# ChanghyeonKim93/nonlinear_optimizer_for_slam

Measured on AMD Instinct MI355X. Metric: ndt6_gauss_newton_residual_blocks_per_sec, higher is better.
Workload: dtype f64

## Files before the change

### nonlinear_optimizer_for_slam_amd/csrc/assemble_one_launch.hpp

```cpp
#pragma once

#include "assemble_pass.hpp"

namespace nos {

constexpr size_t kSingleBlockMaxElements = size_t(1024) * 15;

template <typename Problem, typename T, int BLOCK, bool NT>
__device__ __forceinline__ int single_block_loop(const TiledLayout& L, typename Problem::Params& P, uint32_t n_chunks,
                                                 LmDevice& s_lm, double* s_sum, double* __restrict__ cost_history,
                                                 int history_capacity) {
  constexpr int kF = Problem::kFields;
  constexpr int kOut = Problem::kOut;
  const T* __restrict__ base = static_cast<const T*>(L.base);
  int executed = 0;
  while (s_lm.st.done == 0) {
    set_pose(P, &s_lm);
    T acc[kOut];
#pragma unroll
    for (int k = 0; k < kOut; ++k) acc[k] = T(0);
    constexpr uint32_t kRound = (kF * sizeof(T) > 64) ? 2 : 4;
    for (uint32_t c = 0; c < n_chunks; c += kRound) {
      T x[kRound][kF][1];
      uint64_t i0[kRound];
// ... 79 lines not shown
constexpr uint32_t kClusterMaxBlocks = 256;
constexpr unsigned long long kClusterTimeoutTicks = 5000000ull;
constexpr unsigned long long kClusterMailboxTimeoutTicks = kMailboxTimeoutTicks;

struct ClusterCtl {
  unsigned int abort;
  unsigned int pad0[31];
  struct alignas(128) Arrival {
    unsigned int count;
    unsigned int pad[31];
  } arrival[8];
};

__device__ __forceinline__ double sc1_load(const double* p) {
  return __hip_atomic_load(p, __ATOMIC_RELAXED, __HIP_MEMORY_SCOPE_AGENT);
}
__device__ __forceinline__ void sc1_store(double* p, double v) {
  __hip_atomic_store(p, v, __ATOMIC_RELAXED, __HIP_MEMORY_SCOPE_AGENT);
}

__device__ __forceinline__ void state_store_sc1(LmDevice* lm, const nos_host::LmState& st) {
  double* d = reinterpret_cast<double*>(&lm->st);
  const double* s = reinterpret_cast<const double*>(&st);
  constexpr int kWords = int(sizeof(nos_host::LmState) / sizeof(double));
  static_assert(sizeof(nos_host::LmState) % sizeof(double) == 0, "LmState must be a whole number of doubles");
#pragma unroll
  for (int k = 0; k < kWords; ++k) sc1_store(d + k, s[k]);
}
__device__ __forceinline__ void state_load_sc1(const LmDevice* lm, nos_host::LmState& st) {
  const double* d = reinterpret_cast<const double*>(&lm->st);
  double* s = reinterpret_cast<double*>(&st);
  constexpr int kWords = int(sizeof(nos_host::LmState) / sizeof(double));
#pragma unroll
  for (int k = 0; k < kWords; ++k) s[k] = sc1_load(d + k);
}

template <int FIELDS, int ELEM>
struct ResidentShape;
template <>
struct ResidentShape<15, 8> { static constexpr int RI = 3, LI = 3; };
template <>
struct ResidentShape<15, 4> { static constexpr int RI = 3, LI = 4; };
template <>
struct ResidentShape<5, 8> { static constexpr int RI = 9, LI = 7; };
template <>
struct ResidentShape<5, 4> { static constexpr int RI = 10, LI = 14; };

template <typename Problem, typename T>
struct StreamRegRounds { static constexpr int kRR = 3; };
template <int LOSS>
struct StreamRegRounds<Ndt6Problem<float, LOSS>, float> { static constexpr int kRR = 0; };
constexpr int kStreamRegRoundsMax = 3;

template <typename Problem, typename T, int BLOCK, int RI, int LI, int SI = 0, bool SPF = false, bool NT = false>
__global__ __launch_bounds__(BLOCK) void solve_cluster_kernel(TiledLayout L, typename Problem::Params P,
                                                             double* __restrict__ partials, LmDevice* lm, ClusterCtl* ctl,
                                                             double* __restrict__ cost_history, int history_capacity,
                                                             double* entry_host, unsigned long long* seq_host,
                                                             unsigned long long seq, uint32_t items_per_lane,
                                                             const Mailbox* mail = nullptr, uint32_t stream_lds = 0u,
                                                             uint32_t stream_reg = 0u) {
  constexpr int kF = Problem::kFields;
  constexpr int kOut = Problem::kOut;
  constexpr int kCols = 32;
  constexpr int kSlices = BLOCK / kCols;
  const T* __restrict__ base = static_cast<const T*>(L.base);
  constexpr int kRF = kF;
  extern __shared__ __align__(16) unsigned char resident_raw[];
  T* resident = reinterpret_cast<T*>(resident_raw);
  __shared__ int s_flag;
  __shared__ int s_fast;
  __shared__ double red[kSlices][kCols];
  __shared__ double s_tot[kLmTotDoubles(kOut)];
  __shared__ double s_lmd_raw[(sizeof(LmDevice) + 7) / 8];
  LmDevice& s_lmd = *reinterpret_cast<LmDevice*>(s_lmd_raw);
  nos_host::LmState& s_state = s_lmd.st;
  [[maybe_unused]] __shared__ double s_local[kCols];
  [[maybe_unused]] __shared__ unsigned long long s_round0;
  const bool multi = mail != nullptr;

  const uint32_t J = items_per_lane & 0x7fffffffu;
  [[maybe_unused]] const bool allow_fast = (items_per_lane >> 31) == 0u;
  [[maybe_unused]] constexpr int kXccCol = 28;
  [[maybe_unused]] const unsigned int my_xcc = xcc_id();
  const uint64_t block_base = uint64_t(blockIdx.x) * BLOCK * J;
  auto fetch = [&](uint32_t j, T (&dst)[kRF]) -> bool {
    const uint64_t i = block_base + uint64_t(j) * BLOCK + threadIdx.x;
    const bool ok = i < L.n;
    const uint64_t ic = ok ? i : 0;
    const uint64_t off = (ic >> L.tile_shift) * L.tile_stride + (ic & L.tile_mask);
    T xt[kF][1];
#pragma unroll
    for (int f = 0; f < kF; ++f) load_items<T, 1, false>(base + field_offset<Problem>(L, ic, off, f), xt[f]);
#pragma unroll
    for (int f = 0; f < kF; ++f) dst[f] = ok ? xt[f][0] : T(0);
    return ok;
  };
  auto evaluate_resident = [&](const T (&xi)[kRF], bool ok, T (&acc_)[kOut]) { Problem::item(xi, P, ok, acc_); };
  T x[RI > 0 ? RI : 1][kRF];
  bool valid[RI > 0 ? RI : 1];
  static_assert(SI == 0 || (RI == 0 && LI == 0), "the streaming form keeps nothing resident");
  constexpr int kSI = SI > 0 ? SI : 1;
  [[maybe_unused]] T xs[kF][kSI];
  [[maybe_unused]] uint64_t xs_i0 = 0;
  [[maybe_unused]] constexpr int kRR = (SI > 0 && !SPF) ? StreamRegRounds<Problem, T>::kRR : 0;
  static_assert(kRR <= kStreamRegRoundsMax, "the option's range covers every instantiation");
  [[maybe_unused]] T xr[kRR > 0 ? kRR : 1][kF][kSI];
  [[maybe_unused]] const uint32_t my_rounds = blockIdx.x < J ? (J - blockIdx.x + gridDim.x - 1) / gridDim.x : 0u;
  [[maybe_unused]] const uint32_t lds_k = SI > 0 ? min(stream_lds, my_rounds > 0u ? my_rounds - 1u : 0u) : 0u;
  [[maybe_unused]] const uint32_t reg_k = kRR > 0 ? min(min(stream_reg, uint32_t(kRR)), (my_rounds > 0u ? my_rounds - 1u : 0u) - lds_k) : 0u;
  [[maybe_unused]] const uint32_t alt_k = min(lds_k, reg_k);
  [[maybe_unused]] auto chip_round = [&](uint32_t i) -> uint32_t {
    return uint32_t(uint64_t(i + 1u) * my_rounds / (lds_k + reg_k + 1u));
  };
  [[maybe_unused]] auto lds_slot_round = [&](uint32_t sl) -> uint32_t {
    return sl < lds_k ? chip_round(sl < alt_k ? 2u * sl : alt_k + sl) : ~0u;
  };
  [[maybe_unused]] const uint32_t lds_r0 = lds_slot_round(0u);
  [[maybe_unused]] const uint32_t lds_r1 = lds_slot_round(1u);
  [[maybe_unused]] const uint32_t lds_r2 = lds_slot_round(2u);
  [[maybe_unused]] uint32_t reg_r[kRR > 0 ? kRR : 1];
#pragma unroll
  for (int j = 0; j < (kRR > 0 ? kRR : 1); ++j)
    reg_r[j] = uint32_t(j) < reg_k ? chip_round(uint32_t(j) < alt_k ? 2u * uint32_t(j) + 1u : alt_k + uint32_t(j)) : ~0u;
#pragma unroll
  for (int j = 0; j < (kRR > 0 ? kRR : 1); ++j)
#pragma unroll
    for (int f = 0; f < kF; ++f)
#pragma unroll
      for (int e = 0; e < kSI; ++e) xr[j][f][e] = T(0);
  [[maybe_unused]] auto lds_round = [&](uint32_t s) -> uint32_t { return s == 0u ? lds_r0 : s == 1u ? lds_r1 : s == 2u ? lds_r2 : ~0u; };
  [[maybe_unused]] auto fetch_chunk = [&](uint32_t c, T (&dst)[kF][kSI]) -> uint64_t {
    const uint64_t i0 = uint64_t(c) * (uint64_t(BLOCK) * kSI) + uint64_t(threadIdx.x) * kSI;
    const uint64_t off = (i0 >> L.tile_shift) * L.tile_stride + (i0 & L.tile_mask);
#pragma unroll
    for (int f = 0; f < kF; ++f) load_items<T, kSI, NT>(base + field_offset<Problem>(L, i0, off, f), dst[f]);
    return i0;
  };
  if constexpr (SI > 0) {
    if (blockIdx.x < J) xs_i0 = fetch_chunk(blockIdx.x, xs);
  }
#pragma unroll
  for (int j = 0; j < RI; ++j) {
    valid[j] = false;
    if (uint32_t(j) < J) {
      valid[j] = fetch(uint32_t(j), x[j]);
    } else {
#pragma unroll
      for (int f = 0; f < kRF; ++f) x[j][f] = T(0);
    }
  }
  if constexpr (LI > 0) {
    for (uint32_t j = RI; j < J; ++j) {
      T xi[kRF];
      (void)fetch(j, xi);
#pragma unroll
      for (int f = 0; f < kRF; ++f) resident[(size_t(j - RI) * kRF + f) * BLOCK + threadIdx.x] = xi[f];
    }
  }
  NOS_PROBE(if (threadIdx.x < 4) s_step_cycles[threadIdx.x] = 0ull;)
  if (threadIdx.x == 0) {
    s_lmd.settings = lm->settings;
    s_state = lm->st;
    s_flag = s_state.done != 0 ? 1 : 0;
    s_fast = 0;
    if (__hip_atomic_load(&ctl->abort, __ATOMIC_RELAXED, __HIP_MEMORY_SCOPE_AGENT) != 0u) s_flag = 2;
    if (multi && blockIdx.x == 0) s_round0 = *mail->round;
  }
  __syncthreads();
  [[maybe_unused]] const unsigned int group = blockIdx.x & 7u;
  const unsigned int n_groups = gridDim.x < 8u ? gridDim.x : 8u;
  unsigned int it = 0;
  int executed = 0;
  NOS_PROBE(unsigned long long tq[6] = {0, 0, 0, 0, 0, 0}, tp = 0;)
#define NOS_RES_STAMP(slot_) NOS_PROBE({ const unsigned long long now_ = wall_clock64(); tq[slot_] += now_ - tp; tp = now_; })
  while (s_flag == 0) {
    NOS_PROBE(tp = wall_clock64();)
    if constexpr (kOut == 28) {
#pragma unroll
      for (int k = 0; k < 9; ++k) P.R[k] = T(uniform_load(&s_state.R[k]));
#pragma unroll
      for (int k = 0; k < 3; ++k) P.t[k] = T(uniform_load(&s_state.t[k]));
    } else {
#pragma unroll
      for (int k = 0; k < 4; ++k) P.R2[k] = T(uniform_load(&s_state.R[k]));
#pragma unroll
      for (int k = 0; k < 2; ++k) P.t2[k] = T(uniform_load(&s_state.t[k]));
    }
    T acc[kOut];
#pragma unroll
    for (int k = 0; k < kOut; ++k) acc[k] = T(0);
    if constexpr (SI > 0) {
      const uint32_t n_chunks = J;
      auto evaluate = [&](const T (&xc)[kF][SI > 0 ? SI : 1], uint64_t i0) {
#pragma unroll
        for (int it = 0; it < (SI > 0 ? SI : 1); ++it) {
          T xi[kF];
#pragma unroll
          for (int f = 0; f < kF; ++f) xi[f] = xc[f][it];
          Problem::item(xi, P, (i0 + it) < L.n, acc);
        }
      };
      if constexpr (SPF) {
        for (uint32_t c = blockIdx.x; c < n_chunks; c += gridDim.x) {
          T xb[kF][SI > 0 ? SI : 1];
          uint64_t i1 = 0;
          const uint32_t cn = c + gridDim.x;
          if (cn < n_chunks) i1 = fetch_chunk(cn, xb);
          evaluate(xs, xs_i0);
#pragma unroll
          for (int f = 0; f < kF; ++f)
#pragma unroll
            for (int it = 0; it < (SI > 0 ? SI : 1); ++it) xs[f][it] = xb[f][it];
          xs_i0 = i1;
        }
      } else {
        auto lds_at = [&](uint32_t s, int f, int e) -> T& {
          return resident[((size_t(s) * kF + f) * BLOCK + threadIdx.x) * kSI + e];
        };
        auto evaluate_lds = [&](uint32_t s, uint32_t cl) {
          const uint64_t i0 = uint64_t(cl) * (uint64_t(BLOCK) * kSI) + uint64_t(threadIdx.x) * kSI;
#pragma unroll
          for (int e = 0; e < kSI; ++e) {
            T xi[kF];
#pragma unroll
            for (int f = 0; f < kF; ++f) xi[f] = lds_at(s, f, e);
            Problem::item(xi, P, (i0 + e) < L.n, acc);
          }
        };
        const bool on_chip = it != 0u;
        uint32_t s = 0;
        uint32_t next_res = lds_round(0u);
        auto in_registers = [&](uint32_t r) -> bool {
          bool hit = false;
#pragma unroll
          for (int j = 0; j < kRR; ++j) hit = hit || r == reg_r[j];
          return hit;
        };
        uint32_t k = 0;
        if constexpr (kRR == 0) {
          while (k < my_rounds) {
            __builtin_amdgcn_sched_barrier(0);
            if (!on_chip && k == next_res) {
#pragma unroll
              for (int f = 0; f < kF; ++f)
#pragma unroll
                for (int e = 0; e < kSI; ++e) lds_at(s, f, e) = xs[f][e];
              next_res = lds_round(++s);
            }
            evaluate(xs, xs_i0);
            uint32_t kn = k + 1u;
            if (on_chip)
              for (uint32_t sn = s; kn == lds_round(sn); ++sn) ++kn;
            xs_i0 = fetch_chunk(blockIdx.x + (kn < my_rounds ? kn : 0u) * gridDim.x, xs);
            for (uint32_t kr = k + 1u; kr < kn; ++kr) {
              evaluate_lds(s, blockIdx.x + kr * gridDim.x);
              next_res = lds_round(++s);
            }
            k = kn;
          }
        } else
#pragma unroll
        for (int j = 0; j <= kRR; ++j) {
          const uint32_t rj = j < kRR ? reg_r[j < kRR ? j : 0] : ~0u;
          const uint32_t stop = min(rj, my_rounds);
          const uint32_t hi = (!on_chip && rj != ~0u) ? rj + 1u : stop;
          auto lds_rounds_below = [&](uint32_t lim) {
            while (next_res < lim) {
              evaluate_lds(s, blockIdx.x + next_res * gridDim.x);
              next_res = lds_round(++s);
            }
          };
          if (on_chip && j > 0) lds_rounds_below(min(k, stop));
          while (k < hi) {
            __builtin_amdgcn_sched_barrier(0);
            if (!on_chip) {
              if (k == next_res) {
#pragma unroll
                for (int f = 0; f < kF; ++f)
#pragma unroll
                  for (int e = 0; e < kSI; ++e) lds_at(s, f, e) = xs[f][e];
                next_res = lds_round(++s);
              }
              if constexpr (kRR > 0) {
                if (j < kRR && k == rj) {
#pragma unroll
                  for (int f = 0; f < kF; ++f)
#pragma unroll
                    for (int e = 0; e < kSI; ++e) xr[j < kRR ? j : 0][f][e] = xs[f][e];
                }
              }
            }
            evaluate(xs, xs_i0);
            uint32_t kn = k + 1u;
            if (on_chip) {
              for (uint32_t sn = s;;) {
                if (kn == lds_round(sn)) {
                  ++sn;
                  ++kn;
                } else if (in_registers(kn)) {
                  ++kn;
                } else {
                  break;
                }
              }
            }
            xs_i0 = fetch_chunk(blockIdx.x + (kn < my_rounds ? kn : 0u) * gridDim.x, xs);
            if (on_chip) lds_rounds_below(min(kn, stop));
            k = kn;
          }
          if constexpr (kRR > 0) {
            if (j < kRR && on_chip && rj != ~0u)
              evaluate(xr[j < kRR ? j : 0], uint64_t(blockIdx.x + rj * gridDim.x) * (uint64_t(BLOCK) * kSI) + uint64_t(threadIdx.x) * kSI);
          }
        }
      }
      if constexpr (SPF) {
        if (blockIdx.x < n_chunks) xs_i0 = fetch_chunk(blockIdx.x, xs);
      }
    } else
    if (sizeof(T) == 8 && J >= uint32_t(RI)) {
#pragma unroll
      for (int j = 0; j < RI; ++j) evaluate_resident(x[j], valid[j], acc);
    } else {
#pragma unroll
      for (int j = 0; j < RI; ++j)
        if (uint32_t(j) < J) evaluate_resident(x[j], valid[j], acc);
    }
    if constexpr (LI > 0) {
      for (uint32_t j = RI; j < J; ++j) {
        T xi[kRF];
#pragma unroll
        for (int f = 0; f < kRF; ++f) xi[f] = resident[(size_t(j - RI) * kRF + f) * BLOCK + threadIdx.x];
        evaluate_resident(xi, (block_base + uint64_t(j) * BLOCK + threadIdx.x) < L.n, acc);
      }
    }
    double dacc[kOut];
#pragma unroll
    for (int k = 0; k < kOut; ++k) dacc[k] = double(acc[k]);
    NOS_RES_STAMP(0)
    {
      TaggedUnit* const block_units = reinterpret_cast<TaggedUnit*>(partials);
      TaggedUnit* const group_units = block_units + size_t(kClusterMaxBlocks) * 32;
      const unsigned long long tag = (seq << 24) | ((unsigned long long)it + 1ull);
      const double mine = block_reduce_value<kOut, BLOCK>(dacc);
      const bool probe = it == 0u && allow_fast;
      if (threadIdx.x < kOut) {
        if (s_fast != 0)
          tagged_store_plain(block_units + size_t(blockIdx.x) * 32 + threadIdx.x, mine, tag);
        else
          tagged_store(block_units + size_t(blockIdx.x) * 32 + threadIdx.x, mine, tag);
      } else if (probe && threadIdx.x == kXccCol) {
        tagged_store(block_units + size_t(blockIdx.x) * 32 + kXccCol, double(my_xcc), tag);
      }
      NOS_RES_STAMP(1)
      const unsigned long long deadline = wall_clock64() + (multi ? kClusterMailboxTimeoutTicks : kClusterTimeoutTicks);
      auto await = [&](const TaggedUnit* u, double* value) -> bool {
        unsigned int polls = 0;
        for (;;) {
          const TaggedUnit got = tagged_load(u);
          if (got.seq == tag) {
            *value = got.value;
            return true;
          }
          if ((++polls & 63u) == 0u &&
              (__hip_atomic_load(&ctl->abort, __ATOMIC_RELAXED, __HIP_MEMORY_SCOPE_AGENT) != 0u || wall_clock64() > deadline)) {
            __hip_atomic_store(&ctl->abort, 1u, __ATOMIC_RELAXED, __HIP_MEMORY_SCOPE_AGENT);
// ... 73 lines not shown
                const unsigned long long* slot_r = own + (size_t(r) * 2 + parity) * kMailSlotDoubles;
                unsigned long long got = 0ull;
                unsigned int polls = 0;
                for (;;) {
                  if (lane < 2 * kOut) got = __hip_atomic_load(slot_r + lane, __ATOMIC_RELAXED, __HIP_MEMORY_SCOPE_SYSTEM);
                  const bool here = lane >= 2 * kOut || (unsigned int)(got >> 32) == xtag;
                  if (__ballot(!here) == 0ull) break;
                  if ((++polls & 15u) == 0u) {
                    const unsigned long long peer_gave_up =
                        __hip_atomic_load(slot_r + 63, __ATOMIC_RELAXED, __HIP_MEMORY_SCOPE_SYSTEM);
                    if ((unsigned int)(peer_gave_up >> 32) == xtag || wall_clock64() > give_up_at ||
                        __hip_atomic_load(&ctl->abort, __ATOMIC_RELAXED, __HIP_MEMORY_SCOPE_AGENT) != 0u) {
                      lost = true;
                      break;
                    }
                  }
                  __builtin_amdgcn_s_sleep(1);
                }
                const unsigned int half = (unsigned int)(got & 0xFFFFFFFFull);
                const unsigned int other = (unsigned int)__shfl_xor(int(half), 1, kWave);
                const double value = __longlong_as_double((long long)(((unsigned long long)((lane & 1) ? half : other) << 32) |
                                                                      (unsigned long long)((lane & 1) ? other : half)));
                sum += value;
              }
              if (lost) {
                if (lane == 0) {
                  __hip_atomic_store(&ctl->abort, 1u, __ATOMIC_RELAXED, __HIP_MEMORY_SCOPE_AGENT);
                  s_flag = 2;
                }
                if (lane < mb.n_ranks)
                  __hip_atomic_store(reinterpret_cast<unsigned long long*>(mb.peers[lane] + units_base) +
                                         (size_t(mb.rank) * 2 + parity) * kMailSlotDoubles + 63,
                                     (unsigned long long)xtag << 32, __ATOMIC_RELAXED, __HIP_MEMORY_SCOPE_SYSTEM);
              } else if (lane < 2 * kOut && (lane & 1) == 0) {
                s_local[lane >> 1] = sum;
              }
            }
          }
          __syncthreads();
          if (s_flag != 2) {
            if (threadIdx.x < kOut || (probe && threadIdx.x == kXccCol))
              tagged_store(global_units + size_t(it & 1u) * 32 + threadIdx.x, s_local[threadIdx.x], tag);
          }
        }
        {
          double v = 0.0;
          if (threadIdx.x < kCols && (col < kOut || (probe && col == kXccCol)) && s_flag != 2)
            (void)await(global_units + size_t(it & 1u) * 32 + col, &v);
          if (threadIdx.x < kCols) red[0][col] = v;
        }
        __syncthreads();
      }
      NOS_RES_STAMP(2)
      if (s_flag == 2) break;
      if (multi) {
        if (threadIdx.x < kOut)
          s_tot[threadIdx.x] = red[0][threadIdx.x];
        else if (probe && threadIdx.x == kXccCol)
          s_fast = red[0][kXccCol] == 0.0 ? 1 : 0;
      } else
      if (threadIdx.x < kOut) {
        double tot = 0.0;
        for (unsigned int g = 0; g < n_groups; ++g) tot += red[g][threadIdx.x];
        s_tot[threadIdx.x] = tot;
      } else if (probe && threadIdx.x == kXccCol) {
        double strangers = 0.0;
        for (unsigned int g = 0; g < n_groups; ++g) strangers += red[g][kXccCol];
        s_fast = strangers == 0.0 ? 1 : 0;
      }
      __syncthreads();
    }
    {
      NOS_RES_STAMP(3)
      if (threadIdx.x == 0) {
        if (blockIdx.x == 0 && cost_history != nullptr && executed < history_capacity)
          __hip_atomic_store(cost_history + executed, s_tot[kOut - 1], __ATOMIC_RELAXED, __HIP_MEMORY_SCOPE_SYSTEM);
        lm_step_lane<kOut>(lds_ptr(s_tot), lds_ptr(&s_lmd));
        s_flag = s_state.done != 0 ? 1 : 0;
      }
    }
    ++executed;
    ++it;
    __syncthreads();
    NOS_RES_STAMP(4)
  }
  NOS_PROBE(
  if (blockIdx.x == 0 && threadIdx.x == 0 && entry_host != nullptr) {
    for (int k = 0; k < 5; ++k)
      __hip_atomic_store(entry_host + 50 + k, double(tq[k]) / double(executed > 0 ? executed : 1), __ATOMIC_RELAXED,
                         __HIP_MEMORY_SCOPE_SYSTEM);
    for (int k = 0; k < 3; ++k)
      __hip_atomic_store(entry_host + 56 + k, double(s_step_cycles[k]) / double(executed > 0 ? executed : 1), __ATOMIC_RELAXED,
                         __HIP_MEMORY_SCOPE_SYSTEM);
  }
  )
  if (s_flag == 1 && blockIdx.x == 0) {
    if (threadIdx.x < kOut && entry_host != nullptr && executed > 0)
      __hip_atomic_store(entry_host + kLogOut + threadIdx.x, s_tot[threadIdx.x], __ATOMIC_RELAXED, __HIP_MEMORY_SCOPE_SYSTEM);
    if (threadIdx.x == 0) {
      const nos_host::LmState st = s_state;
      lm->st = st;
      if (multi) *mail->round = s_round0 + (unsigned long long)executed;
      if (entry_host != nullptr) {
#pragma unroll
        for (int k = 0; k < 9; ++k)
          __hip_atomic_store(entry_host + kLogR + k, st.R[k], __ATOMIC_RELAXED, __HIP_MEMORY_SCOPE_SYSTEM);
#pragma unroll
        for (int k = 0; k < 3; ++k)
          __hip_atomic_store(entry_host + kLogT + k, st.t[k], __ATOMIC_RELAXED, __HIP_MEMORY_SCOPE_SYSTEM);
        __hip_atomic_store(entry_host + kLogLambda, st.lambda, __ATOMIC_RELAXED, __HIP_MEMORY_SCOPE_SYSTEM);
        __hip_atomic_store(entry_host + kLogPrevCost, st.previous_cost, __ATOMIC_RELAXED, __HIP_MEMORY_SCOPE_SYSTEM);
        __hip_atomic_store(entry_host + kLogCost, st.cost, __ATOMIC_RELAXED, __HIP_MEMORY_SCOPE_SYSTEM);
        __hip_atomic_store(entry_host + kLogIteration, double(st.iteration), __ATOMIC_RELAXED, __HIP_MEMORY_SCOPE_SYSTEM);
        __hip_atomic_store(entry_host + kLogDone, double(st.done), __ATOMIC_RELAXED, __HIP_MEMORY_SCOPE_SYSTEM);
        __hip_atomic_store(entry_host + kLogOk, double(st.ok), __ATOMIC_RELAXED, __HIP_MEMORY_SCOPE_SYSTEM);
        __hip_atomic_store(entry_host + kLogExecuted, double(executed), __ATOMIC_RELAXED, __HIP_MEMORY_SCOPE_SYSTEM);
      }
    }
    if (threadIdx.x < kWave) {
      asm volatile("s_waitcnt vmcnt(0)" ::: "memory");
      if (threadIdx.x == 0 && seq_host != nullptr) {
        __builtin_amdgcn_fence(__ATOMIC_RELEASE, "");
        asm volatile("s_waitcnt vmcnt(0)" ::: "memory");
        __hip_atomic_store(seq_host, seq, __ATOMIC_RELAXED, __HIP_MEMORY_SCOPE_SYSTEM);
      }
    }
  }
}

}
```

### nonlinear_optimizer_for_slam_amd/csrc/nos_core.hip

```cpp
#include "nos_internal.hpp"

namespace nosd {


thread_local const void* t_last_kernel = nullptr;

template <typename Problem, typename T, int ITEMS, int BLOCK, int MINW, int PREFETCH = 0>
int launch_variant(const nos::TiledLayout& L, const typename Problem::Params& P, int grid_cap, int num_cus_hint,
                   bool nt, double* partials, const nos::FusedFinal& fin_in, hipStream_t stream, int* rows_out) {
  constexpr uint32_t kChunk = BLOCK * ITEMS;
  if (L.n_padded % kChunk != 0) return fail(NOS_ERR_INVALID_ARGUMENT, "n_padded %% chunk != 0");
  if (L.tile_stride != 0 && ((size_t(L.tile_mask) + 1) % kChunk) != 0)
    return fail(NOS_ERR_INVALID_ARGUMENT, "tile not a multiple of the kernel chunk");
  const uint64_t n_chunks64 = L.n_padded / kChunk;
  if (n_chunks64 > 0xFFFFFFFFull) return fail(NOS_ERR_UNSUPPORTED, "dataset too large for one shard");
  const uint32_t n_chunks = uint32_t(n_chunks64);
  int grid = int(std::min<uint64_t>(n_chunks, uint64_t(grid_cap)));
  if (grid < 1) grid = 1;
  if (grid > kMaxPartialRows) grid = kMaxPartialRows;
  nos::FusedFinal fin = fin_in;
  fin.write_through = (fin.counter != nullptr && grid <= num_cus_hint && fin_in.write_through != 0) ? 1 : 0;
  const auto kernel = nt ? nos::assemble_kernel<Problem, T, ITEMS, BLOCK, MINW, true, PREFETCH>
                         : nos::assemble_kernel<Problem, T, ITEMS, BLOCK, MINW, false, PREFETCH>;
  t_last_kernel = reinterpret_cast<const void*>(kernel);
// ... 25 lines not shown
  if constexpr (sizeof(T) == 8) {
    if (variant == 0 && kReproj) variant = 7;
    switch (variant) {
      NOS_CASE(0, 1, 512, 3, 1)
      NOS_CASE(1, 1, 256, 3, 2)
      NOS_CASE(3, 2, 256, 2, 2)
      NOS_CASE_PP(7, 1, 512, kReproj ? 3 : 2, 1)
#ifdef NOS_ALL_VARIANTS
      NOS_CASE(2, 1, 256, 2, 2)
      NOS_CASE(4, 2, 512, 2, 1)
      NOS_CASE_PP(8, 2, 512, 2, 1)
#endif
    }
  } else {
    if (variant == 0) variant = kReproj ? 11 : 1;
    switch (variant) {
      NOS_CASE(1, 2, 512, 2, 1)
      NOS_CASE_PP(11, 2, 512, 2, 1)
#ifdef NOS_ALL_VARIANTS
      NOS_CASE(2, 1, 256, 4, 2)
      NOS_CASE(3, 2, 256, 5, 2)
      NOS_CASE(4, 2, 256, 4, 2)
      NOS_CASE(5, 1, 1024, 4, 1)
      NOS_CASE(6, 2, 1024, 4, 1)
      NOS_CASE(9, 2, 256, 3, 3)
      NOS_CASE_PP(12, 4, 512, 2, 1)
      NOS_CASE(13, 4, 256, 2, 1)
#endif
    }
  }
#undef NOS_CASE
#undef NOS_CASE_PP
  return fail(NOS_ERR_UNSUPPORTED, "launch geometry %d is not compiled into this build for this element type "
              "(default build: fp64 0, 1, 3, 7; fp32 1, 11; `make ALL_VARIANTS=1` builds the rest)", variant);
}

size_t resident_items_per_lane(int n_fields, int dtype) {
  if (n_fields == 15)
    return dtype == NOS_F64 ? size_t(nos::ResidentShape<15, 8>::RI + nos::ResidentShape<15, 8>::LI)
                            : size_t(nos::ResidentShape<15, 4>::RI + nos::ResidentShape<15, 4>::LI);
  if (n_fields == 5)
    return dtype == NOS_F64 ? size_t(nos::ResidentShape<5, 8>::RI + nos::ResidentShape<5, 8>::LI)
                            : size_t(nos::ResidentShape<5, 4>::RI + nos::ResidentShape<5, 4>::LI);
  return 1;
}

struct SingleBlockArgs {
  int cluster_blocks = 0;
  int items_per_lane = 1;
  int stream_chunks = 0;
  bool nt = false;
  int stream_lds_chunks = 0;
  int stream_reg_rounds = 0;
  bool stage1_sc1 = false;
  const nos::Mailbox* mail = nullptr;
  double* partials = nullptr;
  nos::ClusterCtl* ctl = nullptr;
  nos::LmDevice* lm;
  double* history;
  int history_capacity;
  double* entry;
  unsigned long long* seq_host;
  unsigned long long seq;
};

template <typename Problem, typename T>
int launch_single(const nos::TiledLayout& L, const typename Problem::Params& P, const SingleBlockArgs& a, hipStream_t stream) {
  constexpr int kBlock = 512;
  if (L.n_padded % kBlock != 0) return fail(NOS_ERR_INVALID_ARGUMENT, "n_padded %% 512 != 0");
  if (a.cluster_blocks > 0 && a.stream_chunks > 0) {
    constexpr int kSI = sizeof(T) == 8 ? 1 : 2;
    constexpr bool kSPF = false;
    constexpr size_t kChunk = size_t(kBlock) * kSI;
    if (L.n_padded % kChunk != 0 || (L.tile_stride != 0 && ((size_t(L.tile_mask) + 1) % kChunk) != 0))
      return fail(NOS_ERR_INVALID_ARGUMENT, "streaming solve: layout not a multiple of the %zu-item chunk", kChunk);
    if (size_t(a.stream_chunks) * kChunk != L.n_padded) return fail(NOS_ERR_INVALID_ARGUMENT, "streaming solve: chunk count does not match the layout");
    const auto kernel = a.nt ? nos::solve_cluster_kernel<Problem, T, kBlock, 0, 0, kSI, kSPF, true>
                             : nos::solve_cluster_kernel<Problem, T, kBlock, 0, 0, kSI, kSPF, false>;
    uint32_t lds = uint32_t(std::min(std::max(a.stream_lds_chunks, 0), 3));
    size_t dyn_bytes = lds * size_t(Problem::kFields) * kChunk * sizeof(T);
    if (dyn_bytes > size_t(48) * 1024 &&
        hipFuncSetAttribute(reinterpret_cast<const void*>(kernel), hipFuncAttributeMaxDynamicSharedMemorySize,
                            int(dyn_bytes)) != hipSuccess) {
      (void)hipGetLastError();
      lds = 0;
      dyn_bytes = 0;
    }
    const uint32_t reg = uint32_t(std::min(std::max(a.stream_reg_rounds, 0), nos::kStreamRegRoundsMax));
    t_last_kernel = reinterpret_cast<const void*>(kernel);
    hipLaunchKernelGGL(kernel, dim3(a.cluster_blocks), dim3(kBlock), dyn_bytes, stream, L, P, a.partials, a.lm, a.ctl, a.history,
                       a.history_capacity, a.entry, a.seq_host, a.seq, uint32_t(a.stream_chunks) | (a.stage1_sc1 ? 0x80000000u : 0u),
                       a.mail, lds, reg);
    hipError_t e = hipGetLastError();
    if (e != hipSuccess) return fail(NOS_ERR_HIP, "streaming solve launch failed: %s", hipGetErrorString(e));
    return NOS_OK;
  }
  if (a.cluster_blocks > 0) {
    using Shape = nos::ResidentShape<Problem::kPlanes, int(sizeof(T))>;
    if (a.items_per_lane < 1 || a.items_per_lane > Shape::RI + Shape::LI)
      return fail(NOS_ERR_INVALID_ARGUMENT, "resident solve: %d items per lane do not fit (%d + %d)", a.items_per_lane,
                  Shape::RI, Shape::LI);
    const auto kernel = nos::solve_cluster_kernel<Problem, T, kBlock, Shape::RI, Shape::LI>;
    const size_t lds_items = a.items_per_lane > Shape::RI ? size_t(a.items_per_lane - Shape::RI) : 0;
    const size_t dyn_bytes = lds_items * size_t(Problem::kFields) * kBlock * sizeof(T);
    if (dyn_bytes > size_t(48) * 1024) {
      const hipError_t ea = hipFuncSetAttribute(reinterpret_cast<const void*>(kernel),
                                                hipFuncAttributeMaxDynamicSharedMemorySize, int(dyn_bytes));
      if (ea != hipSuccess) return fail(NOS_ERR_UNSUPPORTED, "resident solve: %zu bytes of LDS refused: %s", dyn_bytes, hipGetErrorString(ea));
    }
    t_last_kernel = reinterpret_cast<const void*>(kernel);
    hipLaunchKernelGGL(kernel, dim3(a.cluster_blocks), dim3(kBlock), dyn_bytes, stream, L, P, a.partials, a.lm, a.ctl,
                       a.history, a.history_capacity, a.entry, a.seq_host, a.seq,
                       uint32_t(a.items_per_lane) | (a.stage1_sc1 ? 0x80000000u : 0u), a.mail, 0u, 0u);
    hipError_t e = hipGetLastError();
    if (e != hipSuccess) return fail(NOS_ERR_HIP, "cluster solve launch failed: %s", hipGetErrorString(e));
    return NOS_OK;
  }
  const uint32_t n_chunks = uint32_t((std::max<uint64_t>(L.n, 1) + kBlock - 1) / kBlock);
  t_last_kernel = reinterpret_cast<const void*>(&nos::solve_single_block_kernel<Problem, T, kBlock>);
  hipLaunchKernelGGL((nos::solve_single_block_kernel<Problem, T, kBlock>), dim3(1), dim3(kBlock), 0, stream, L, P, n_chunks, a.lm,
                     a.history, a.history_capacity, a.entry, a.seq_host, a.seq);
  hipError_t e = hipGetLastError();
  if (e != hipSuccess) return fail(NOS_ERR_HIP, "single-workgroup solve launch failed: %s", hipGetErrorString(e));
  return NOS_OK;
}

template <template <typename, int> class ProblemT, typename T, typename ParamsT>
int launch_by_loss(int loss_kind, int variant, int blocks_per_cu, int num_cus,
                   const nos::TiledLayout& L, const ParamsT& P, bool nt, double* partials,
                   const nos::FusedFinal& fin, hipStream_t stream, int* rows_out, const SingleBlockArgs* single = nullptr) {
  return with_loss(loss_kind, [&](auto loss) {
    using Problem = ProblemT<T, decltype(loss)::value>;
    if (single) return launch_single<Problem, T>(L, P, *single, stream);
    return launch_by_variant<Problem, T>(variant, blocks_per_cu, num_cus, L, P, nt, partials, fin, stream, rows_out);
  });
}

int check_loss(const nos_loss* loss, int* kind_out) {
  int kind = loss ? loss->kind : NOS_LOSS_NONE;
  if (kind < NOS_LOSS_NONE || kind > NOS_LOSS_HUBER) return fail(NOS_ERR_INVALID_ARGUMENT, "unknown loss kind %d", kind);
  if (kind == NOS_LOSS_EXPONENTIAL && (loss->a < 0.0 || loss->b < 0.0))
    return fail(NOS_ERR_INVALID_ARGUMENT, "exponential loss needs c1 >= 0 and c2 >= 0");
  if (kind == NOS_LOSS_HUBER && !(loss->a > 0.0)) return fail(NOS_ERR_INVALID_ARGUMENT, "huber loss needs threshold > 0");
  *kind_out = kind;
  return NOS_OK;
}

bool use_nontemporal(const nos_dataset* ds, const Shard& sh) {
  const int force = ds->ctx->settings.nt;
  if (force >= 0) return force != 0;
  return sh.bytes > (size_t(192) << 20);
}

template <template <typename, int> class ProblemT, typename T>
int launch_flat(const nos_dataset* ds, const Shard& sh, const Request& rq, double* partials, const nos::FusedFinal& fin,
                hipStream_t stream, int* rows_out, const SingleBlockArgs* single) {
  const nos_ctx* ctx = ds->ctx;
  typename ProblemT<T, nos::kLossNone>::Params P{};
  fill_params(P, rq, ds);
  return launch_by_loss<ProblemT, T>(rq.loss_kind, ctx->variant, ctx->blocks_per_cu, ctx->slots[sh.slot].num_cus, sh.layout, P,
                                     use_nontemporal(ds, sh), partials, fin, stream, rows_out, single);
}

int launch_assemble_inner(const nos_dataset* ds, const Shard& sh, const Request& rq, double* partials,
                          const nos::FusedFinal& fin_in, hipStream_t stream, int* rows_out, const SingleBlockArgs* single) {
  nos::FusedFinal fin = fin_in;
// ... 316 lines not shown
  const int executed = int(e[nos::kLogExecuted]);
  if (slot.prof_on && slot.prof_every == 0) slot.prof_launches += executed;
  copy_history(opt, slot, executed);
  return NOS_OK;
}

bool cluster_eligible(const nos_dataset* ds, const nos_lm_options* opt, bool mailbox_in_launch, size_t cluster_blocks,
                      bool resident_fits, bool stream_form, bool paused) {
  const nos_ctx* ctx = ds->ctx;
  const bool with_comm = ctx->comm != nullptr;
  return ds->kind != kKindNdtIndexed && !with_comm && (ctx->shm_dev == nullptr || mailbox_in_launch) && opt->max_iterations > 0 &&
         cluster_blocks >= 1 && (resident_fits || stream_form) && !paused &&
         ctx->settings.lm_cluster != 0 && (opt->cost_history == nullptr || opt->max_iterations <= kHistCapacity);
}

int solve_cluster(nos_dataset* ds, const Request& rq, const nos_lm_options* opt, const nos::LmInitArgs& init,
                  nos_host::LmState* st, bool* finished, int* fell_back) {
  nos_ctx* ctx = ds->ctx;
  const Shard& sh = ds->shards[0];
  DeviceSlot& slot = ctx->slots[sh.slot];
  *finished = false;
  const size_t max_blocks = std::min<size_t>(std::min<size_t>(nos::kClusterMaxBlocks, size_t(slot.num_cus)),
                                             size_t(std::max(1, ctx->settings.lm_cluster_max_blocks)));
  const bool mailbox_in_launch = ctx->shm_dev != nullptr && ctx->d_peers != nullptr && ctx->d_mail != nullptr &&
                                 ds->kind != kKindNdtIndexed;
  const size_t cluster_blocks = std::min<size_t>(max_blocks, (sh.layout.n + 511) / 512);
  const size_t items_per_lane = cluster_blocks > 0 ? (sh.layout.n + cluster_blocks * 512 - 1) / (cluster_blocks * 512) : 0;
  const size_t resident_capacity = ctx->settings.lm_cluster == 2 ? 1 : resident_items_per_lane(ds->n_fields, ds->dtype);
  const size_t stream_chunk = size_t(512) * (ds->dtype == NOS_F64 ? 1 : 2);
  const bool resident_fits = items_per_lane >= 1 && items_per_lane <= resident_capacity;
  const bool stream_form = !resident_fits && (ctx->settings.lm_cluster == 1 || ctx->settings.lm_cluster == 5) && items_per_lane >= 1 &&
                           sh.layout.n_padded % stream_chunk == 0 && sh.layout.n_padded / stream_chunk < (size_t(1) << 31) &&
                           (sh.layout.tile_stride == 0 || (size_t(sh.layout.tile_mask) + 1) % stream_chunk == 0);
  bool paused = false;
  if (mailbox_in_launch) {
    paused = slot.cluster_paused_solves > 0;
    if (paused) --slot.cluster_paused_solves;
  } else {
    if (slot.cluster_gave_up &&
        std::chrono::steady_clock::now() - slot.cluster_gave_up_at > std::chrono::milliseconds(ctx->settings.lm_cluster_retry_ms))
      slot.cluster_gave_up = false;
    paused = slot.cluster_gave_up;
  }
  if (!cluster_eligible(ds, opt, mailbox_in_launch, cluster_blocks, resident_fits, stream_form, paused)) return NOS_OK;
  SingleBlockArgs cl{};
  cl.cluster_blocks = int(cluster_blocks);
  cl.items_per_lane = int(items_per_lane);
  if (stream_form) {
    cl.items_per_lane = 0;
    cl.stream_chunks = int(sh.layout.n_padded / stream_chunk);
    cl.nt = use_nontemporal(ds, sh);
    cl.stream_lds_chunks = ctx->settings.stream_lds_chunks;
    cl.stream_reg_rounds = ctx->settings.stream_reg_rounds;
  }
  cl.stage1_sc1 = ctx->settings.lm_cluster == 5;
  cl.mail = mailbox_in_launch ? ctx->d_mail : nullptr;
  cl.partials = slot.partials;
  cl.ctl = slot.d_cluster;
  cl.lm = slot.d_lm;
  cl.history = opt->cost_history ? slot.h_hist_dev : nullptr;
  cl.history_capacity = kHistCapacity;
  cl.entry = slot.h_log_dev;
  cl.seq_host = reinterpret_cast<unsigned long long*>(slot.h_out_dev + kSeqSlot);
  cl.seq = ++slot.seq;
  NOS_HIP_CHECK(hipMemsetAsync(slot.d_cluster, 0, sizeof(nos::ClusterCtl), slot.stream));
  if (ctx->settings.debug_cluster_abort != 0) {
    const unsigned int raised = 1u;
    NOS_HIP_CHECK(hipMemcpyAsync(&slot.d_cluster->abort, &raised, sizeof raised, hipMemcpyHostToDevice, slot.stream));
    NOS_HIP_CHECK(hipStreamSynchronize(slot.stream));
  }
  int rows = 0;
  const int rc_launch = launch_assemble_raw(ds, sh, rq, slot.partials, nos::FusedFinal{}, slot.stream, &rows, &cl);
  if (rc_launch != NOS_OK && rc_launch != NOS_ERR_UNSUPPORTED) return rc_launch;
  const bool launched_ok = rc_launch == NOS_OK;
  *finished = launched_ok && spin_for_sequence(slot, cl.seq, 4000000);
  if (!*finished) {
    NOS_HIP_CHECK(hipStreamSynchronize(slot.stream));
    *finished = spin_for_sequence(slot, cl.seq, 1);
  }
  if (*finished) {
    slot.cluster_next_pause = 64;
    const double* e = slot.h_log;
    read_log_entry(e, st);
    const int executed = int(e[nos::kLogExecuted]);
#ifdef NOS_LM_TIMING
    fprintf(stderr, "[resident-timing] %d blocks x %d items/lane (0 = streamed), %d iterations; workgroup 0, us per iteration: item math %.2f, "
            "block reduce %.2f, drain+arrive+wait %.2f, rows->sums %.2f, LM step+barrier %.2f\n", cl.cluster_blocks,
            cl.items_per_lane, executed, e[50] * 0.01, e[51] * 0.01, e[52] * 0.01, e[53] * 0.01, e[54] * 0.01);
    fprintf(stderr, "[resident-timing]    inside the step, shader-clock cycles per iteration: elimination %.0f, back substitution %.0f, "
            "lane 0 (pose update, tests, schedule) %.0f\n", e[56], e[57], e[58]);
#endif
    if (slot.prof_on && slot.prof_every == 0) slot.prof_launches += executed;
    copy_history(opt, slot, executed);
    return NOS_OK;
  }
  *fell_back = 1;
  if (launched_ok && ctx->settings.debug_cluster_abort != 1) {
    if (mailbox_in_launch) {
      slot.cluster_paused_solves = slot.cluster_next_pause;
      slot.cluster_next_pause = std::min(slot.cluster_next_pause * 2, 65536);
    } else {
      slot.cluster_gave_up = true;
      slot.cluster_gave_up_at = std::chrono::steady_clock::now();
    }
  }
  if (!launched_ok) clear_last_error();
// ... 243 lines not shown
```

### nonlinear_optimizer_for_slam_amd/csrc/nos_ctx.hip

```cpp
#include "nos_internal.hpp"

#include <cxxabi.h>

namespace nosd {

namespace {
thread_local std::string g_last_error;
}

int fail(int status, const char* fmt, ...) {
  char buf[512];
  va_list ap;
  va_start(ap, fmt);
  vsnprintf(buf, sizeof buf, fmt, ap);
  va_end(ap);
  g_last_error = buf;
  return status;
}

const char* last_error_text() { return g_last_error.c_str(); }
void clear_last_error() { g_last_error.clear(); }

std::string dir_of_symbol(const void* symbol, std::string* file_out) {
  Dl_info info{};
// ... 50 lines not shown
void pool_release(DeviceSlot& slot, void* ptr, size_t capacity) {
  if (!ptr) return;
  if (!slot.pool_enabled || capacity > kPoolMaxBytes) {
    (void)hipFree(ptr);
    return;
  }
  slot.pool.push_back({ptr, capacity});
  slot.pool_bytes += capacity;
  while (slot.pool.size() > kPoolMaxEntries || slot.pool_bytes > kPoolMaxBytes) {
    (void)hipFree(slot.pool.front().ptr);
    slot.pool_bytes -= slot.pool.front().bytes;
    slot.pool.erase(slot.pool.begin());
  }
}

}

using namespace nosd;

namespace {
struct OptionEntry {
  const char* key;
  int nosd::Settings::*field;
  int lo, hi;
};
const OptionEntry kOptions[] = {
    {"plane_skew", &nosd::Settings::plane_skew, 0, 1 << 20},
    {"sc1", &nosd::Settings::sc1, 0, 1},
    {"nt", &nosd::Settings::nt, -1, 1},
    {"fused", &nosd::Settings::fused, 0, 1},
    {"lm_fused", &nosd::Settings::lm_fused, 0, 1},
    {"lm_window", &nosd::Settings::lm_window, 1, nosd::kLogSlots - 2},
    {"lm_single", &nosd::Settings::lm_single, 0, 1},
    {"lm_cluster", &nosd::Settings::lm_cluster, 0, 5},
    {"lm_cluster_retry_ms", &nosd::Settings::lm_cluster_retry_ms, 0, 3600000},
    {"pool", &nosd::Settings::pool, 0, 1},
    {"tile_log2", &nosd::Settings::tile_log2, -1, 24},
    {"ingest", &nosd::Settings::ingest, 0, 2},
    {"ingest_threads", &nosd::Settings::ingest_threads, 0, 1024},
    {"indexed_bpc", &nosd::Settings::indexed_bpc, 1, 16},
    {"match_dense", &nosd::Settings::match_dense, 0, 1},
    {"map_compact_keys", &nosd::Settings::map_compact_keys, 0, 1},
    {"pgo_host_scalars", &nosd::Settings::pgo_host_scalars, 0, 1},
    {"pgo_precond", &nosd::Settings::pgo_precond, 0, 1},
    {"pgo_agg", &nosd::Settings::pgo_agg, 2, 1 << 20},
    {"pgo_block", &nosd::Settings::pgo_block, 0, 1},
    {"pgo_coarse_probe", &nosd::Settings::pgo_coarse_probe, 0, 1},
    {"map_fma_mask", &nosd::Settings::map_fma_mask, 0, (1 << 26) - 1},
    {"map_eigen_version", &nosd::Settings::map_eigen_version, 33, 34},
    {"debug_cluster_abort", &nosd::Settings::debug_cluster_abort, 0, 2},
    {"lm_cluster_max_blocks", &nosd::Settings::lm_cluster_max_blocks, 1, 256},
    {"stream_lds_chunks", &nosd::Settings::stream_lds_chunks, 0, 3},
    {"stream_reg_rounds", &nosd::Settings::stream_reg_rounds, 0, nos::kStreamRegRoundsMax},
    {"batch_max_elements", &nosd::Settings::batch_max_elements, 0, 1 << 30},
};
bool option_in_range(const OptionEntry& o, int value) {
  if (value < o.lo || value > o.hi) return false;
  if (!strcmp(o.key, "tile_log2")) return value <= 0 || value >= 10;
  return true;
}
void drop_out_of_range_settings(nosd::Settings& st) {
  const nosd::Settings defaults;
  for (const OptionEntry& o : kOptions)
    if (!option_in_range(o, st.*(o.field))) {
      fprintf(stderr, "[nos-hip] NOS_%s = %d is outside [%d, %d]: ignored\n", o.key, st.*(o.field), o.lo, o.hi);
      st.*(o.field) = defaults.*(o.field);
    }
}
}


extern "C" {

int nos_ctx_create(const int* device_ids, int n_devices, nos_ctx** out_ctx) {
  if (!out_ctx) return fail(NOS_ERR_INVALID_ARGUMENT, "out_ctx is NULL");
  *out_ctx = nullptr;
  if (n_devices < 1 || n_devices > 64 || !device_ids) return fail(NOS_ERR_INVALID_ARGUMENT, "bad device list");
  int count = 0;
  hipError_t e = hipGetDeviceCount(&count);
  if (e != hipSuccess || count < 1)
    return fail(NOS_ERR_NO_DEVICE, "no usable HIP device (%s); this library has no CPU fallback",
                e != hipSuccess ? hipGetErrorString(e) : "device count is 0");
  for (int i = 0; i < n_devices; ++i)
    if (device_ids[i] < 0 || device_ids[i] >= count)
      return fail(NOS_ERR_INVALID_ARGUMENT, "device id %d out of range [0,%d)", device_ids[i], count);
  nos_ctx* ctx = new (std::nothrow) nos_ctx();
  if (!ctx) return fail(NOS_ERR_OUT_OF_MEMORY, "host allocation failed");
  ctx->slots.resize(n_devices);
  ctx->blocks_per_cu = env_int("NOS_BLOCKS_PER_CU", 0);
  ctx->variant = env_int("NOS_VARIANT", 0);
  {
    Settings& st = ctx->settings;
    st.plane_skew = env_int("NOS_PLANE_SKEW", st.plane_skew);
    st.sc1 = env_int("NOS_SC1", st.sc1);
    st.nt = env_int("NOS_NT", st.nt);
    st.fused = env_int("NOS_FUSED", st.fused);
    st.lm_fused = env_int("NOS_LM_FUSED", st.lm_fused);
    st.lm_window = env_int("NOS_LM_WINDOW", st.lm_window);
    st.lm_single = env_int("NOS_LM_SINGLE", st.lm_single);
    st.lm_cluster = env_int("NOS_LM_CLUSTER", st.lm_cluster);
    st.lm_cluster_max_blocks = env_int("NOS_LM_CLUSTER_MAX_BLOCKS", st.lm_cluster_max_blocks);
    st.stream_lds_chunks = env_int("NOS_STREAM_LDS_CHUNKS", st.stream_lds_chunks);
    st.stream_reg_rounds = env_int("NOS_STREAM_REG_ROUNDS", st.stream_reg_rounds);
    st.batch_max_elements = env_int("NOS_BATCH_MAX_ELEMENTS", st.batch_max_elements);
    st.pool = env_int("NOS_POOL", st.pool);
    st.tile_log2 = env_int("NOS_TILE_LOG2", st.tile_log2);
    const char* ingest = getenv("NOS_INGEST");
    st.ingest = (ingest && !strcmp(ingest, "pack")) ? 1 : ((ingest && !strcmp(ingest, "unpack")) ? 2 : 0);
    st.ingest_threads = env_int("NOS_INGEST_THREADS", 0);
    st.indexed_bpc = env_int("NOS_INDEXED_BPC", st.indexed_bpc);
    st.match_dense = env_int("NOS_MATCH_DENSE", st.match_dense);
    st.map_compact_keys = env_int("NOS_MAP_COMPACT_KEYS", st.map_compact_keys);
    st.pgo_host_scalars = env_int("NOS_PGO_HOST_SCALARS", st.pgo_host_scalars);
    st.pgo_precond = env_int("NOS_PGO_PRECOND", st.pgo_precond);
    st.pgo_agg = env_int("NOS_PGO_AGG", st.pgo_agg);
    st.pgo_block = env_int("NOS_PGO_BLOCK", st.pgo_block);
    st.pgo_coarse_probe = env_int("NOS_PGO_COARSE_PROBE", st.pgo_coarse_probe);
    drop_out_of_range_settings(st);
  }
  for (int i = 0; i < n_devices; ++i) {
    DeviceSlot& s = ctx->slots[i];
    s.device = device_ids[i];
    s.pool_enabled = ctx->settings.pool != 0;
    hipDeviceProp_t prop;
    e = hipSetDevice(s.device);
    if (e == hipSuccess) e = hipGetDeviceProperties(&prop, s.device);
    if (e == hipSuccess) {
      s.num_cus = prop.multiProcessorCount > 0 ? prop.multiProcessorCount : 256;
      e = hipStreamCreateWithFlags(&s.own_stream, hipStreamNonBlocking);
    }
    if (e == hipSuccess) e = hipMalloc(&s.partials, sizeof(double) * kMaxPartialRows * kMaxOut);
    if (e == hipSuccess) e = hipMalloc(&s.d_out, sizeof(double) * kMaxOut);
    if (e == hipSuccess) e = hipHostMalloc(&s.h_out, sizeof(double) * 64, hipHostMallocMapped);
    if (e == hipSuccess) memset(s.h_out, 0, sizeof(double) * 64);
    if (e == hipSuccess) e = hipHostGetDevicePointer(reinterpret_cast<void**>(&s.h_out_dev), s.h_out, 0);
    if (e == hipSuccess) e = hipMalloc(&s.d_lm, sizeof(nos::LmDevice));
    const size_t log_bytes = sizeof(double) * kLogSlots * nos::kLogEntryDoubles;
    if (e == hipSuccess) e = hipHostMalloc(&s.h_log, log_bytes, hipHostMallocMapped);
    if (e == hipSuccess) memset(s.h_log, 0, log_bytes);
    if (e == hipSuccess) e = hipHostGetDevicePointer(reinterpret_cast<void**>(&s.h_log_dev), s.h_log, 0);
    if (e == hipSuccess) e = hipMalloc(reinterpret_cast<void**>(&s.d_cluster), sizeof(nos::ClusterCtl));
    if (e == hipSuccess) e = hipMemset(s.d_cluster, 0, sizeof(nos::ClusterCtl));
    if (e == hipSuccess) e = hipHostMalloc(&s.h_hist, sizeof(double) * kHistCapacity, hipHostMallocMapped);
    if (e == hipSuccess) e = hipHostGetDevicePointer(reinterpret_cast<void**>(&s.h_hist_dev), s.h_hist, 0);
    if (e == hipSuccess) e = hipMalloc(&s.counter, 2048);
    if (e == hipSuccess) e = hipMemset(s.counter, 0, 2048);
    if (e == hipSuccess) e = hipEventCreate(&s.ev0);
    if (e == hipSuccess) e = hipEventCreate(&s.ev1);
    if (e == hipSuccess) e = hipEventCreate(&s.ev2);
    s.stream = s.own_stream;
    if (e != hipSuccess) {
      nos_ctx_destroy(ctx);
      return fail(e == hipErrorOutOfMemory ? NOS_ERR_OUT_OF_MEMORY : NOS_ERR_HIP, "context setup failed on device %d: %s",
                  device_ids[i], hipGetErrorString(e));
    }
  }
// ... 232 lines not shown
```

### nonlinear_optimizer_for_slam_amd/csrc/nos_internal.hpp

```cpp
#pragma once

#include <hip/hip_runtime.h>
#include <dlfcn.h>
#include <fcntl.h>
#include <sys/mman.h>
#include <sys/stat.h>
#include <unistd.h>
#include <rccl/rccl.h>

#include <algorithm>
#include <atomic>
#include <chrono>
#include <random>
#include <climits>
#include <cmath>
#include <cstdarg>
#include <cstdio>
#include <cstdlib>
#include <cstring>
#include <map>
#include <memory>
#include <new>
#include <string>
#include <thread>
// ... 86 lines not shown
  void* pack_pinned[2] = {nullptr, nullptr};
  size_t pack_bytes = 0;
  void* batch_pinned = nullptr;
  size_t batch_pinned_bytes = 0;
  hipEvent_t pack_done[2] = {nullptr, nullptr};
  struct PoolEntry {
    void* ptr;
    size_t bytes;
  };
  std::vector<PoolEntry> pool;
  size_t pool_bytes = 0;
  bool pool_enabled = true;
  const void* last_kernel = nullptr;
  bool cluster_gave_up = false;
  std::chrono::steady_clock::time_point cluster_gave_up_at{};
  int cluster_paused_solves = 0;
  int cluster_next_pause = 64;
  std::vector<hipEvent_t> prof_events;
  size_t prof_used = 0;
  bool prof_on = false;
  int prof_every = 1;
  long prof_launches = 0;
};

constexpr int kMapReferenceFmaMask = (4 | 8 | 16 | 32) | ((1 | 4 | 8 | 32 | 256) << 8) | (0x1ff << 17);
struct Settings {
  int plane_skew = 1088;
  int sc1 = 1;
  int nt = -1;
  int fused = 1;
  int lm_fused = 1;
  int lm_window = 3;
  int lm_single = 1;
  int lm_cluster_retry_ms = 5000;
  int lm_cluster = 1;
  int pool = 1;
  int tile_log2 = -1;
  int ingest = 0;
  int ingest_threads = 0;
  int indexed_bpc = 1;
  int match_dense = 1;
  int map_compact_keys = 1;
  int pgo_host_scalars = 0;
  int pgo_precond = 1;
  int pgo_agg = 48;
  int pgo_coarse_probe = 0;
  int pgo_block = 1;
  int map_fma_mask = kMapReferenceFmaMask;
  int map_eigen_version = 34;
  int debug_cluster_abort = 0;
  int lm_cluster_max_blocks = 256;
  int stream_lds_chunks = 3;
  int stream_reg_rounds = 3;
  int batch_max_elements = int(nos::kSingleBlockMaxElements);
};
}

struct nos_ctx {
  std::recursive_mutex mu;
  nosd::Settings settings;
  std::vector<nosd::DeviceSlot> slots;
  int blocks_per_cu = 0;
  int variant = 0;
  int tile_log2 = -1;
  ncclComm_t comm = nullptr;
  int comm_ranks = 1;
  int comm_rank = 0;
  void* shm_host = nullptr;
  size_t shm_bytes = 0;
  double* shm_dev = nullptr;
  unsigned long long* d_round = nullptr;
  nos::Mailbox* d_mail = nullptr;
  double* ipc_own = nullptr;
  std::vector<double*> ipc_peers;
  double** d_peers = nullptr;
};

namespace nosd {

struct CtxGuard {
  std::unique_lock<std::recursive_mutex> lock;
  explicit CtxGuard(const nos_ctx* ctx) {
    if (ctx != nullptr) lock = std::unique_lock<std::recursive_mutex>(const_cast<nos_ctx*>(ctx)->mu);
  }
};

struct Shard {
  int slot = 0;
  nos::TiledLayout layout{};
  void* data = nullptr;
  size_t bytes = 0;
  size_t capacity = 0;
  bool pooled = false;
  int32_t* index = nullptr;
  void* table = nullptr;
  bool one_block = false;
  int n_slots = 0;
  size_t n_voxels = 0;
};

}

struct nos_dataset {
  nos_ctx* ctx = nullptr;
  int kind = 0;
  int dtype = NOS_F64;
// ... 249 lines not shown
```

Before: 76.85 billion.

## Prefetch second streamed chunk during LM step to overlap next-iteration loads

Adds a tail-round prefetch: while the block finishes the LM step of one iteration, it fetches the chunk for round 1 into a spare register buffer. The next iteration then evaluates round 0 and swaps in the prefetched data, so the first streamed loads are hidden behind the reduction and solve. It is enabled by default through a new setting and applies only to streaming configurations with register rounds (not float NDT3). The cost is extra register pressure from another chunk buffer and more control-flow complexity.

After: 76.94 billion, median of 5. Within noise of the previous version (+0.1%).

```diff
diff --git a/nonlinear_optimizer_for_slam_amd/csrc/assemble_one_launch.hpp b/nonlinear_optimizer_for_slam_amd/csrc/assemble_one_launch.hpp
--- a/nonlinear_optimizer_for_slam_amd/csrc/assemble_one_launch.hpp
+++ b/nonlinear_optimizer_for_slam_amd/csrc/assemble_one_launch.hpp
@@ -155,6 +155,11 @@
 struct StreamRegRounds<Ndt6Problem<float, LOSS>, float> { static constexpr int kRR = 0; };
 constexpr int kStreamRegRoundsMax = 3;
 
+template <typename Problem, typename T>
+struct StreamTailRound { static constexpr int kTR = StreamRegRounds<Problem, T>::kRR > 0 ? 1 : 0; };
+template <int LOSS>
+struct StreamTailRound<Ndt3Problem<float, LOSS>, float> { static constexpr int kTR = 0; };
+
 template <typename Problem, typename T, int BLOCK, int RI, int LI, int SI = 0, bool SPF = false, bool NT = false>
 __global__ __launch_bounds__(BLOCK) void solve_cluster_kernel(TiledLayout L, typename Problem::Params P,
                                                              double* __restrict__ partials, LmDevice* lm, ClusterCtl* ctl,
@@ -162,7 +167,7 @@
                                                              double* entry_host, unsigned long long* seq_host,
                                                              unsigned long long seq, uint32_t items_per_lane,
                                                              const Mailbox* mail = nullptr, uint32_t stream_lds = 0u,
-                                                             uint32_t stream_reg = 0u) {
+                                                             uint32_t stream_reg = 0u, uint32_t stream_tail = 0u) {
   constexpr int kF = Problem::kFields;
   constexpr int kOut = Problem::kOut;
   constexpr int kCols = 32;
@@ -232,6 +237,11 @@
     for (int f = 0; f < kF; ++f)
 #pragma unroll
       for (int e = 0; e < kSI; ++e) xr[j][f][e] = T(0);
+  [[maybe_unused]] constexpr int kTR = (kRR > 0) ? StreamTailRound<Problem, T>::kTR : 0;
+  [[maybe_unused]] T xb[kF][kSI];
+  [[maybe_unused]] uint64_t xb_i0 = 0;
+  [[maybe_unused]] const bool tail_ok =
+      kTR > 0 && stream_tail != 0u && my_rounds >= 3u && (lds_k + reg_k == 0u || chip_round(0u) != 1u);
   [[maybe_unused]] auto lds_round = [&](uint32_t s) -> uint32_t { return s == 0u ? lds_r0 : s == 1u ? lds_r1 : s == 2u ? lds_r2 : ~0u; };
   [[maybe_unused]] auto fetch_chunk = [&](uint32_t c, T (&dst)[kF][kSI]) -> uint64_t {
     const uint64_t i0 = uint64_t(c) * (uint64_t(BLOCK) * kSI) + uint64_t(threadIdx.x) * kSI;
@@ -306,15 +316,15 @@
       };
       if constexpr (SPF) {
         for (uint32_t c = blockIdx.x; c < n_chunks; c += gridDim.x) {
-          T xb[kF][SI > 0 ? SI : 1];
+          T xn[kF][SI > 0 ? SI : 1];
           uint64_t i1 = 0;
           const uint32_t cn = c + gridDim.x;
-          if (cn < n_chunks) i1 = fetch_chunk(cn, xb);
+          if (cn < n_chunks) i1 = fetch_chunk(cn, xn);
           evaluate(xs, xs_i0);
 #pragma unroll
           for (int f = 0; f < kF; ++f)
 #pragma unroll
-            for (int it = 0; it < (SI > 0 ? SI : 1); ++it) xs[f][it] = xb[f][it];
+            for (int it = 0; it < (SI > 0 ? SI : 1); ++it) xs[f][it] = xn[f][it];
           xs_i0 = i1;
         }
       } else {
@@ -362,7 +372,36 @@
             }
             k = kn;
           }
-        } else
+        } else {
+        auto next_streamed = [&](uint32_t k0) -> uint32_t {
+          uint32_t kn = k0;
+          if (on_chip) {
+            for (uint32_t sn = s;;) {
+              if (kn == lds_round(sn)) {
+                ++sn;
+                ++kn;
+              } else if (in_registers(kn)) {
+                ++kn;
+              } else {
+                break;
+              }
+            }
+          }
+          return kn;
+        };
+        if constexpr (kTR > 0) {
+          if (tail_ok && on_chip) {
+            __builtin_amdgcn_sched_barrier(0);
+            evaluate(xs, xs_i0);
+            __builtin_amdgcn_sched_barrier(0);
+#pragma unroll
+            for (int f = 0; f < kF; ++f)
+#pragma unroll
+              for (int e = 0; e < kSI; ++e) xs[f][e] = xb[f][e];
+            xs_i0 = xb_i0;
+            k = 1u;
+          }
+        }
 #pragma unroll
         for (int j = 0; j <= kRR; ++j) {
           const uint32_t rj = j < kRR ? reg_r[j < kRR ? j : 0] : ~0u;
@@ -374,7 +413,7 @@
               next_res = lds_round(++s);
             }
           };
-          if (on_chip && j > 0) lds_rounds_below(min(k, stop));
+          if (on_chip && (j > 0 || kTR > 0)) lds_rounds_below(min(k, stop));
           while (k < hi) {
             __builtin_amdgcn_sched_barrier(0);
             if (!on_chip) {
@@ -395,19 +434,7 @@
               }
             }
             evaluate(xs, xs_i0);
-            uint32_t kn = k + 1u;
-            if (on_chip) {
-              for (uint32_t sn = s;;) {
-                if (kn == lds_round(sn)) {
-                  ++sn;
-                  ++kn;
-                } else if (in_registers(kn)) {
-                  ++kn;
-                } else {
-                  break;
-                }
-              }
-            }
+            const uint32_t kn = next_streamed(k + 1u);
             xs_i0 = fetch_chunk(blockIdx.x + (kn < my_rounds ? kn : 0u) * gridDim.x, xs);
             if (on_chip) lds_rounds_below(min(kn, stop));
             k = kn;
@@ -416,6 +443,7 @@
             if (j < kRR && on_chip && rj != ~0u)
               evaluate(xr[j < kRR ? j : 0], uint64_t(blockIdx.x + rj * gridDim.x) * (uint64_t(BLOCK) * kSI) + uint64_t(threadIdx.x) * kSI);
           }
+        }
         }
       }
       if constexpr (SPF) {
@@ -595,6 +623,13 @@
         __syncthreads();
       }
       NOS_RES_STAMP(2)
+      if constexpr (kTR > 0) {
+        xb_i0 = 0;
+#pragma unroll
+        for (int f = 0; f < kF; ++f)
+#pragma unroll
+          for (int e = 0; e < kSI; ++e) xb[f][e] = T(0);
+      }
       if (s_flag == 2) break;
       if (multi) {
         if (threadIdx.x < kOut)
@@ -621,6 +656,13 @@
         lm_step_lane<kOut>(lds_ptr(s_tot), lds_ptr(&s_lmd));
         s_flag = s_state.done != 0 ? 1 : 0;
       }
+      if constexpr (kTR > 0) {
+        if (tail_ok) {
+          uint32_t c1 = blockIdx.x + gridDim.x;
+          asm volatile("" : "+s"(c1));
+          xb_i0 = fetch_chunk(c1, xb);
+        }
+      }
     }
     ++executed;
     ++it;
diff --git a/nonlinear_optimizer_for_slam_amd/csrc/nos_core.hip b/nonlinear_optimizer_for_slam_amd/csrc/nos_core.hip
--- a/nonlinear_optimizer_for_slam_amd/csrc/nos_core.hip
+++ b/nonlinear_optimizer_for_slam_amd/csrc/nos_core.hip
@@ -101,6 +101,7 @@
   bool nt = false;
   int stream_lds_chunks = 0;
   int stream_reg_rounds = 0;
+  int stream_tail_round = 0;
   bool stage1_sc1 = false;
   const nos::Mailbox* mail = nullptr;
   double* partials = nullptr;
@@ -139,7 +140,7 @@
     t_last_kernel = reinterpret_cast<const void*>(kernel);
     hipLaunchKernelGGL(kernel, dim3(a.cluster_blocks), dim3(kBlock), dyn_bytes, stream, L, P, a.partials, a.lm, a.ctl, a.history,
                        a.history_capacity, a.entry, a.seq_host, a.seq, uint32_t(a.stream_chunks) | (a.stage1_sc1 ? 0x80000000u : 0u),
-                       a.mail, lds, reg);
+                       a.mail, lds, reg, a.stream_tail_round != 0 ? 1u : 0u);
     hipError_t e = hipGetLastError();
     if (e != hipSuccess) return fail(NOS_ERR_HIP, "streaming solve launch failed: %s", hipGetErrorString(e));
     return NOS_OK;
@@ -160,7 +161,7 @@
     t_last_kernel = reinterpret_cast<const void*>(kernel);
     hipLaunchKernelGGL(kernel, dim3(a.cluster_blocks), dim3(kBlock), dyn_bytes, stream, L, P, a.partials, a.lm, a.ctl,
                        a.history, a.history_capacity, a.entry, a.seq_host, a.seq,
-                       uint32_t(a.items_per_lane) | (a.stage1_sc1 ? 0x80000000u : 0u), a.mail, 0u, 0u);
+                       uint32_t(a.items_per_lane) | (a.stage1_sc1 ? 0x80000000u : 0u), a.mail, 0u, 0u, 0u);
     hipError_t e = hipGetLastError();
     if (e != hipSuccess) return fail(NOS_ERR_HIP, "cluster solve launch failed: %s", hipGetErrorString(e));
     return NOS_OK;
@@ -583,6 +584,7 @@
     cl.nt = use_nontemporal(ds, sh);
     cl.stream_lds_chunks = ctx->settings.stream_lds_chunks;
     cl.stream_reg_rounds = ctx->settings.stream_reg_rounds;
+    cl.stream_tail_round = ctx->settings.stream_tail_round;
   }
   cl.stage1_sc1 = ctx->settings.lm_cluster == 5;
   cl.mail = mailbox_in_launch ? ctx->d_mail : nullptr;
diff --git a/nonlinear_optimizer_for_slam_amd/csrc/nos_ctx.hip b/nonlinear_optimizer_for_slam_amd/csrc/nos_ctx.hip
--- a/nonlinear_optimizer_for_slam_amd/csrc/nos_ctx.hip
+++ b/nonlinear_optimizer_for_slam_amd/csrc/nos_ctx.hip
@@ -126,6 +126,7 @@
     {"lm_cluster_max_blocks", &nosd::Settings::lm_cluster_max_blocks, 1, 256},
     {"stream_lds_chunks", &nosd::Settings::stream_lds_chunks, 0, 3},
     {"stream_reg_rounds", &nosd::Settings::stream_reg_rounds, 0, nos::kStreamRegRoundsMax},
+    {"stream_tail_round", &nosd::Settings::stream_tail_round, 0, 1},
     {"batch_max_elements", &nosd::Settings::batch_max_elements, 0, 1 << 30},
 };
 bool option_in_range(const OptionEntry& o, int value) {
@@ -176,6 +177,7 @@
     st.lm_cluster_max_blocks = env_int("NOS_LM_CLUSTER_MAX_BLOCKS", st.lm_cluster_max_blocks);
     st.stream_lds_chunks = env_int("NOS_STREAM_LDS_CHUNKS", st.stream_lds_chunks);
     st.stream_reg_rounds = env_int("NOS_STREAM_REG_ROUNDS", st.stream_reg_rounds);
+    st.stream_tail_round = env_int("NOS_STREAM_TAIL_ROUND", st.stream_tail_round);
     st.batch_max_elements = env_int("NOS_BATCH_MAX_ELEMENTS", st.batch_max_elements);
     st.pool = env_int("NOS_POOL", st.pool);
     st.tile_log2 = env_int("NOS_TILE_LOG2", st.tile_log2);
diff --git a/nonlinear_optimizer_for_slam_amd/csrc/nos_internal.hpp b/nonlinear_optimizer_for_slam_amd/csrc/nos_internal.hpp
--- a/nonlinear_optimizer_for_slam_amd/csrc/nos_internal.hpp
+++ b/nonlinear_optimizer_for_slam_amd/csrc/nos_internal.hpp
@@ -162,6 +162,7 @@
   int lm_cluster_max_blocks = 256;
   int stream_lds_chunks = 3;
   int stream_reg_rounds = 3;
+  int stream_tail_round = 1;
   int batch_max_elements = int(nos::kSingleBlockMaxElements);
 };
 }
```
